# ardaduz/deep-video-mvs

Measured on NVIDIA H100. Metric: fusionnet depth frames/sec @256x256x64planes, higher is better.
Workload: dtype f16+f32acc

## Files before the change

### deep-video-mvs_b200/dvmvs/_blocks.py

```python
import torch

from . import _native as N
from . import _ops as ops
from ._base import NativeModule, auto_graph, pack_cbr, pack_head
from .config import Config
from .convlstm import MVSLayernormConvLSTMCell
from .layers import conv_layer, depth_layer_3x3

fpn_output_channels = 32
hyper_channels = 32

D, U = N.SRC_DIRECT, N.SRC_UPSAMPLE2X


class StandardLayer(NativeModule):
    def __init__(self, channels, kernel_size, apply_bn_relu):
        super().__init__()
        self.conv1 = conv_layer(channels, channels, kernel_size, 1, True)
        self.conv2 = conv_layer(channels, channels, kernel_size, 1, apply_bn_relu)

    def _pack(self):
        return ops.ConvLayer(pack_cbr(self.conv1)), ops.ConvLayer(pack_cbr(self.conv2))

    def run(self, x):
# ... 72 lines not shown
                depth = depth_producer()
                c1.prestage_upsampled(depth)
        x = self.up_convolution.run(x)
        if fork is not None:
            fork.join()
        srcs = [(x, D), (skip, D)] if depth is None else [(x, D), (skip, D), (depth, U)]
        h, w = x.f32.shape[1], x.f32.shape[2]
        blk_only = c1.path(h, w) == "halo" and c2.path(h, w) == "halo"
        y = c1.run(srcs, want_f32=not blk_only, want_planes=not blk_only)
        return c2.run([(y, D)], want_planes=False, want_blk=False)

    def forward(self, x, skip, depth):
        return ops.act_to_api(self.run(ops.to_act(x), ops.to_act(skip), None if depth is None else ops.to_act(depth)))


class _InvertedResidual(torch.nn.Module):

    def __init__(self, in_ch, out_ch, kernel_size, stride, expansion):
        super().__init__()
        mid = in_ch * expansion
        self.apply_residual = in_ch == out_ch and stride == 1
        self.stride = stride
        self.layers = torch.nn.Sequential(
            torch.nn.Conv2d(in_ch, mid, 1, bias=False), torch.nn.BatchNorm2d(mid), torch.nn.ReLU(inplace=True),
            torch.nn.Conv2d(mid, mid, kernel_size, padding=kernel_size // 2, stride=stride, groups=mid, bias=False),
            torch.nn.BatchNorm2d(mid), torch.nn.ReLU(inplace=True),
            torch.nn.Conv2d(mid, out_ch, 1, bias=False), torch.nn.BatchNorm2d(out_ch))


def _stack(in_ch, out_ch, kernel_size, stride, expansion, repeats):
    blocks = [_InvertedResidual(in_ch, out_ch, kernel_size, stride, expansion)]
    blocks += [_InvertedResidual(out_ch, out_ch, kernel_size, 1, expansion) for _ in range(repeats - 1)]
    return torch.nn.Sequential(*blocks)


class FeatureExtractor(NativeModule):

    def __init__(self):
        super().__init__()
        self.layer1 = torch.nn.Sequential(
            torch.nn.Conv2d(3, 32, 3, padding=1, stride=2, bias=False), torch.nn.BatchNorm2d(32), torch.nn.ReLU(inplace=True),
            torch.nn.Conv2d(32, 32, 3, padding=1, stride=1, groups=32, bias=False), torch.nn.BatchNorm2d(32), torch.nn.ReLU(inplace=True),
            torch.nn.Conv2d(32, 16, 1, padding=0, stride=1, bias=False), torch.nn.BatchNorm2d(16))
        self.layer2 = torch.nn.Sequential(_stack(16, 24, 3, 2, 3, 3))
        self.layer3 = torch.nn.Sequential(_stack(24, 40, 5, 2, 3, 3))
        self.layer4 = torch.nn.Sequential(_stack(40, 80, 5, 2, 6, 3), _stack(80, 96, 3, 1, 6, 2))
        self.layer5 = torch.nn.Sequential(_stack(96, 192, 5, 2, 6, 4), _stack(192, 320, 3, 1, 6, 1))

    def _pack(self):
        l1 = self.layer1
        stem = (ops.ConvLayer(ops.PackedConv(l1[0].weight, None, l1[1], stride=2, act=N.ACT_RELU)),
                ops.PackedDepthwise(l1[3].weight, l1[4], stride=1),
                ops.ConvLayer(ops.PackedConv(l1[6].weight, None, l1[7], stride=1, act=N.ACT_NONE)))
        levels = []
        for layer in (self.layer2, self.layer3, self.layer4, self.layer5):
            blocks = []
            for stack in layer:
                for blk in stack:
                    L = blk.layers
                    blocks.append((ops.ConvLayer(ops.PackedConv(L[0].weight, None, L[1], act=N.ACT_RELU)),
                                   ops.PackedDepthwise(L[3].weight, L[4], stride=blk.stride),
                                   ops.ConvLayer(ops.PackedConv(L[6].weight, None, L[7], act=N.ACT_NONE)), blk.apply_residual))
            levels.append(blocks)
        return stem, levels

    def run(self, x, image_nchw=None, part="all"):
        stem, levels = self.packed()
        def depthwise(t, dw, consumer):
            if consumer.uses_tc():
                return ops.Act(None, ops.dwconv2d(t.f32, dw, want_f32=False, want_planes=True)[1])
            return ops.Act(ops.dwconv2d(t.f32, dw))

        outs = []
        if part != "tail":
            if image_nchw is not None:
                x = ops.Act(ops.stem_conv(image_nchw, stem[0].pc))
            else:
                x = stem[0].run([(x, D)])
            x = depthwise(x, stem[1], stem[2])
            x = stem[2].run([(x, D)])
            outs = [x]
        for blocks in {"all": levels, "head": levels[:2], "tail": levels[2:]}[part]:
            for expand, dw, project, residual in blocks:
                y = depthwise(expand.run([(x, D)], want_planes=False), dw, project)
                x = project.run([(y, D)], residual=x if residual else None,
                                residual_mode=N.RES_SAME if residual else N.RES_NONE)
            outs.append(x)
        return outs

    @auto_graph
    @ops.family_terms("fe")
    def forward(self, image):
        B, C, H, W = image.shape
        if C != 3 or H % 32 != 0 or W % 32 != 0:
            raise RuntimeError("FeatureExtractor: expected (B,3,H,W) with H, W multiples of 32, got %s" % (tuple(image.shape),))
        ops.require_cuda_f32(image, "image")
        if image.is_contiguous():
            return tuple(ops.act_to_api(t) for t in self.run(None, image_nchw=image))
        return tuple(ops.act_to_api(t) for t in self.run(ops.to_act(image, "image")))

    @ops.family_terms("fe")
    def forward_head(self, image):
        ops.require_cuda_f32(image, "image")
        return tuple(ops.act_to_api(t) for t in self.run(None, image_nchw=image.contiguous(), part="head"))

    @ops.family_terms("fe")
    def forward_tail(self, head):
        l1, l2, l3 = head
        tail = self.run(ops.to_act(l3, "layer3"), part="tail")
        return (l1, l2, l3) + tuple(ops.act_to_api(t) for t in tail)


class _FPNHolder(torch.nn.Module):

    def __init__(self, in_channels_list, out_channels):
        super().__init__()
        self.inner_blocks = torch.nn.ModuleList([torch.nn.Conv2d(c, out_channels, 1) for c in in_channels_list])
        self.layer_blocks = torch.nn.ModuleList([torch.nn.Conv2d(out_channels, out_channels, 3, padding=1) for _ in in_channels_list])


class FeatureShrinker(NativeModule):

    def __init__(self):
        super().__init__()
        self.fpn = _FPNHolder([16, 24, 40, 96, 320], fpn_output_channels)

    def _pack(self):
        inner = [ops.ConvLayer(ops.PackedConv(m.weight, m.bias)) for m in self.fpn.inner_blocks]
        layer = [ops.ConvLayer(ops.PackedConv(m.weight, m.bias)) for m in self.fpn.layer_blocks]
        return inner, layer

    def run(self, feats):
        inner, layer = self.packed()
        last = inner[4].run([(feats[4], D)])
        outs = [None] * 4
        keep, forks = [last], []
        for i in (3, 2, 1, 0):
            last = inner[i].run([(feats[i], D)], residual=last, residual_mode=N.RES_NEAREST_UP)
            keep.append(last)
            if i > 0:
                f = ops.Fork()
                with f:
                    outs[i] = layer[i].run([(last, D)])
                forks.append(f)
            else:
                outs[i] = layer[i].run([(last, D)])
        for f in forks:
            f.join()
        del keep
        return outs

    @auto_graph
    @ops.family_terms("fpn")
    def forward(self, layer1, layer2, layer3, layer4, layer5):
        feats = [ops.to_act(t, "layer%d" % (i + 1)) for i, t in enumerate((layer1, layer2, layer3, layer4, layer5))]
        return tuple(ops.act_to_api(t) for t in self.run(feats))


class CostVolumeEncoder(NativeModule):
    def __init__(self):
        super().__init__()
        h = hyper_channels
        self.aggregator0 = conv_layer(Config.train_n_depth_levels + fpn_output_channels, h, 5, 1, True)
        self.encoder_block0 = EncoderBlock(h, h * 2, 5)
        self.aggregator1 = conv_layer(h * 2 + fpn_output_channels, h * 2, 3, 1, True)
        self.encoder_block1 = EncoderBlock(h * 2, h * 4, 3)
        self.aggregator2 = conv_layer(h * 4 + fpn_output_channels, h * 4, 3, 1, True)
# ... 113 lines not shown
```

### deep-video-mvs_b200/dvmvs/_native.py

```python
import ctypes
import os

_HERE = os.path.dirname(os.path.abspath(__file__))
LIB_PATH = os.path.join(os.path.dirname(_HERE), "lib", "libdvmvs_sm90.so")

c_float_p = ctypes.c_void_p
ABI_VERSION = 6
_lib = None

ACT_NONE, ACT_RELU, ACT_SIGMOID = 0, 1, 2
SRC_DIRECT, SRC_UPSAMPLE2X = 0, 1
SPLIT_UPSAMPLE2X, SPLIT_HI_ONLY = 1, 2
RES_NONE, RES_SAME, RES_NEAREST_UP = 0, 1, 2
SWEEP_DOT, SWEEP_SAD = 0, 1
LOSS_L1, LOSS_L1_INV, LOSS_L1_REL, LOSS_HUBER = 0, 1, 2, 3

EXPORTED_SYMBOLS = [
    "dvmvs_abi_version", "dvmvs_set_programmatic_launch", "dvmvs_last_error_string", "dvmvs_kernel_launch_count", "dvmvs_plane_sweep_fused",
    "dvmvs_hidden_warp", "dvmvs_depth_reproject", "dvmvs_conv2d", "dvmvs_conv2d_tc", "dvmvs_conv2d_halo", "dvmvs_split_blocked", "dvmvs_split_planes", "dvmvs_stem_conv", "dvmvs_dwconv2d", "dvmvs_lstm_gates",
    "dvmvs_upsample2x", "dvmvs_nchw_to_nhwc", "dvmvs_nhwc_to_nchw", "dvmvs_preprocess_rgb", "dvmvs_tsdf_integrate",
    "dvmvs_plane_sweep_backward", "dvmvs_hidden_warp_backward", "dvmvs_lstm_gates_backward", "dvmvs_depth_loss_forward",
    "dvmvs_depth_loss_backward", "dvmvs_plane_sweep_fused_h16", "dvmvs_plane_sweep_tc", "dvmvs_lstm_gates_parts", "dvmvs_conv2d_tc_ksplit", "dvmvs_plane_sweep_tc_set_timeline",
    "dvmvs_mesh_scratch_bytes", "dvmvs_mesh_count", "dvmvs_mesh_extract",
]


class ConvDesc(ctypes.Structure):
    _fields_ = [
        ("src", ctypes.c_void_p * 3), ("src_channels", ctypes.c_int * 3), ("src_mode", ctypes.c_int * 3),
        ("n_src", ctypes.c_int),
        ("weight", ctypes.c_void_p), ("bias", ctypes.c_void_p), ("residual", ctypes.c_void_p),
        ("residual_mode", ctypes.c_int), ("Hr", ctypes.c_int), ("Wr", ctypes.c_int),
        ("out", ctypes.c_void_p), ("aux_out", ctypes.c_void_p),
        ("aux_mult", ctypes.c_float), ("aux_base", ctypes.c_float),
        ("B", ctypes.c_int), ("Hin", ctypes.c_int), ("Win", ctypes.c_int), ("Cout", ctypes.c_int),
        ("ksize", ctypes.c_int), ("stride", ctypes.c_int), ("act", ctypes.c_int),
        ("workspace", ctypes.c_void_p), ("workspace_bytes", ctypes.c_longlong),
    ]


class ConvTcDesc(ctypes.Structure):
    _fields_ = [
        ("src_planes", ctypes.c_void_p * 3), ("src_channels", ctypes.c_int * 3), ("n_src", ctypes.c_int),
        ("w_hi", ctypes.c_void_p), ("w_lo", ctypes.c_void_p),
        ("w_rows", ctypes.c_int), ("ktot", ctypes.c_int), ("block_n", ctypes.c_int), ("terms", ctypes.c_int),
        ("allow_split", ctypes.c_int),
        ("bias", ctypes.c_void_p), ("residual", ctypes.c_void_p),
        ("residual_mode", ctypes.c_int), ("Hr", ctypes.c_int), ("Wr", ctypes.c_int),
        ("out_f32", ctypes.c_void_p), ("out_planes", ctypes.c_void_p), ("aux_out", ctypes.c_void_p),
        ("aux_mult", ctypes.c_float), ("aux_base", ctypes.c_float),
        ("B", ctypes.c_int), ("Hin", ctypes.c_int), ("Win", ctypes.c_int), ("Cout", ctypes.c_int),
        ("ksize", ctypes.c_int), ("stride", ctypes.c_int), ("act", ctypes.c_int),
        ("workspace", ctypes.c_void_p), ("workspace_bytes", ctypes.c_longlong),
        ("out_blk", ctypes.c_void_p),
        ("out_hi_only", ctypes.c_int), ("defer_finish", ctypes.c_int),
    ]


DRYRUN = os.environ.get("DVMVS_DRYRUN") == "1"


class _DryRunLib:

    def __getattr__(self, name):
        if name == "dvmvs_last_error_string":
            return lambda: b"dry run"
        if name == "dvmvs_kernel_launch_count":
            return lambda: 0
        return lambda *a, **k: 0


class ConvHaloDesc(ctypes.Structure):
    _fields_ = [
        ("src_blk", ctypes.c_void_p * 3), ("src_c8", ctypes.c_int * 3), ("n_src", ctypes.c_int),
        ("w_hi", ctypes.c_void_p), ("w_lo", ctypes.c_void_p),
        ("n_groups", ctypes.c_int), ("kc", ctypes.c_int), ("block_n", ctypes.c_int), ("terms", ctypes.c_int),
        ("bias", ctypes.c_void_p), ("residual", ctypes.c_void_p),
        ("out_f32", ctypes.c_void_p), ("out_blk", ctypes.c_void_p), ("out_nhwc", ctypes.c_void_p),
        ("B", ctypes.c_int), ("H", ctypes.c_int), ("W", ctypes.c_int), ("Cout", ctypes.c_int),
        ("ksize", ctypes.c_int), ("act", ctypes.c_int),
        ("w_cat", ctypes.c_void_p),
        ("out_hi_only", ctypes.c_int),
    ]


def lib():
    global _lib
    if _lib is None and DRYRUN:
        _lib = _DryRunLib()
    if _lib is None:
        if not os.path.isfile(LIB_PATH):
            raise RuntimeError("dvmvs: %s not found -- build it with `python deep-video-mvs_b200/build_native.py` "
                               "(there is no CPU / eager fallback)" % LIB_PATH)
        L = ctypes.CDLL(LIB_PATH)
        if L.dvmvs_abi_version() != ABI_VERSION:
            raise RuntimeError("dvmvs: %s has ABI version %d, this binding was written for %d -- rebuild it with "
                               "`python deep-video-mvs_b200/build_native.py --force`" % (LIB_PATH, L.dvmvs_abi_version(), ABI_VERSION))
        i, f, p = ctypes.c_int, ctypes.c_float, ctypes.c_void_p
        L.dvmvs_last_error_string.restype = ctypes.c_char_p
        L.dvmvs_set_programmatic_launch.argtypes = [i]
        L.dvmvs_plane_sweep_fused.argtypes = [p, p, p, p, p, p, i, i, i, i, i, i, f, f, i, p]
        L.dvmvs_plane_sweep_generic.argtypes = [p, p, p, p, p, p, i, i, i, i, i, i, f, f, i, p]
        L.dvmvs_plane_sweep_fused_h16.argtypes = [p, p, p, p, p, p, i, i, i, i, i, i, f, f, p]
        L.dvmvs_plane_sweep_tc.argtypes = [p, p, p, p, p, p, p, p, i, i, i, i, i, f, f, i, p]
        L.dvmvs_plane_sweep_tc_set_timeline.argtypes = [p]
        L.dvmvs_hidden_warp.argtypes = [p, p, p, p, p, p, i, i, i, i, f, p]
        L.dvmvs_depth_reproject.argtypes = [p, p, p, p, p, p, i, i, i, p]
        L.dvmvs_conv2d.argtypes = [ctypes.POINTER(ConvDesc), p]
        L.dvmvs_conv2d_tc.argtypes = [ctypes.POINTER(ConvTcDesc), p]
        L.dvmvs_conv2d_halo.argtypes = [ctypes.POINTER(ConvHaloDesc), p]
        L.dvmvs_split_blocked.argtypes = [p, p, i, i, i, i, i, i, i, i, p]
        L.dvmvs_split_planes.argtypes = [p, p, i, i, i, i, i, i, i, i, p]
        L.dvmvs_stem_conv.argtypes = [p, p, p, p, i, i, i, p]
        L.dvmvs_dwconv2d.argtypes = [p, p, p, p, p, i, i, i, i, i, i, i, p]
        L.dvmvs_lstm_gates.argtypes = [p, p, p, p, i, i, i, i, p]
        L.dvmvs_lstm_gates_parts.argtypes = [p, i, ctypes.c_longlong, p, p, p, p, i, i, i, i, p]
        L.dvmvs_conv2d_tc_ksplit.argtypes = [ctypes.POINTER(ConvTcDesc)]
        L.dvmvs_upsample2x.argtypes = [p, p, i, i, i, i, p]
        L.dvmvs_preprocess_rgb.argtypes = [p, i, i, i, i, i, i, p, i, i, i, f, ctypes.POINTER(ctypes.c_float), ctypes.POINTER(ctypes.c_float), p]
        L.dvmvs_nchw_to_nhwc.argtypes = [p, p, i, i, i, i, p]
        L.dvmvs_nhwc_to_nchw.argtypes = [p, p, i, i, i, i, p]
        d = ctypes.c_double
        L.dvmvs_tsdf_integrate.argtypes = [p, p, p, i, i, i, ctypes.POINTER(ctypes.c_float), d, d, p, i, p, i, i, i,
                                           ctypes.POINTER(ctypes.c_float), ctypes.POINTER(ctypes.c_double), d, p, p]
        ll = ctypes.c_longlong
        L.dvmvs_mesh_scratch_bytes.argtypes = [i, i, i, ctypes.POINTER(ll)]
        L.dvmvs_mesh_count.argtypes = [p, i, i, i, p, ll, p]
        L.dvmvs_mesh_extract.argtypes = [p, p, i, i, i, ctypes.POINTER(ctypes.c_float), f, p, ll, i, i, p, p, p, p, p, p]
        L.dvmvs_plane_sweep_backward.argtypes = [p, p, p, p, p, p, p, p, i, i, i, i, i, i, f, f, i, p]
        L.dvmvs_hidden_warp_backward.argtypes = [p, p, p, p, p, p, i, i, i, i, f, p]
        L.dvmvs_lstm_gates_backward.argtypes = [p, p, p, p, p, p, i, i, i, i, p]
        ip, fp = ctypes.POINTER(ctypes.c_int), ctypes.POINTER(ctypes.c_float)
        L.dvmvs_depth_loss_forward.argtypes = [p, ip, ip, i, p, p, i, i, i, p]
        L.dvmvs_depth_loss_backward.argtypes = [p, p, ip, ip, fp, i, p, p, p, i, i, i, i, p]
        _lib = L
    return _lib


def check(rc, what):
    if rc != 0:
        raise RuntimeError("dvmvs native call %s failed (%d): %s" % (what, rc, lib().dvmvs_last_error_string().decode()))


def launch_count():
    return lib().dvmvs_kernel_launch_count()
```

### deep-video-mvs_b200/dvmvs/_ops.py

```python
import ctypes
import os as _os_mod


def _os_environ_get(k, d):
    return _os_mod.environ.get(k, d)


import torch

from . import _native as N


def _stream():
    if N.DRYRUN:
        return None
    return ctypes.c_void_p(torch.cuda.current_stream().cuda_stream)


def _first_tensor(args):
    for a in args:
        if isinstance(a, torch.Tensor):
            return a
        if isinstance(a, (list, tuple)):
            t = _first_tensor(a)
# ... 389 lines not shown
        w2d = torch.zeros(rows, self.ktot, dtype=torch.float32)
        w2d[:cout] = wk.reshape(self.ktot, cout).t()
        hi = w2d.to(torch.float16)
        lo = (w2d - hi.to(torch.float32)).to(torch.float16)
        self.w_hi = hi.contiguous().to(device)
        self.w_lo = lo.contiguous().to(device)
        self.rows = rows
        self.ksize, self.cin, self.cout, self.stride, self.act = k, cin, cout, pc.stride, pc.act
        self.bias = pc.bias.to(device) if pc.bias is not None else None
        self.src_channels = list(src_channels)


@on_tensor_device
def conv2d_tc(sources, ptc, residual=None, residual_mode=N.RES_NONE, aux=None, want_f32=True, want_planes=True, terms=3,
              block_n=None, allow_split=True, blk_out=None, defer_finish=False):
    d = N.ConvTcDesc()
    first = sources[0]
    B, Hin, Win = first.shape[1], first.shape[2], first.shape[3]
    if len(sources) != len(ptc.src_stored):
        raise ValueError("conv2d_tc: %d sources given, weights packed for %d" % (len(sources), len(ptc.src_stored)))
    for i, t in enumerate(sources):
        if t.dtype != torch.float16 or tuple(t.shape[:4]) != (2, B, Hin, Win) or t.shape[4] != ptc.src_stored[i]:
            raise ValueError("conv2d_tc: source %d has shape %s / %s, expected (2,%d,%d,%d,%d) fp16"
                             % (i, tuple(t.shape), t.dtype, B, Hin, Win, ptc.src_stored[i]))
        d.src_planes[i] = t.data_ptr()
        d.src_channels[i] = t.shape[4]
    d.n_src = len(sources)
    pad = (ptc.ksize - 1) // 2
    Hout = (Hin + 2 * pad - ptc.ksize) // ptc.stride + 1
    Wout = (Win + 2 * pad - ptc.ksize) // ptc.stride + 1
    if block_n is None:
        tiles = B * ((Hout + 7) // 8) * ((Wout + 15) // 16)
        if ptc.cout >= 1024 and tiles < 16:
            block_n = 128
        elif ptc.cout <= 32 or tiles < 16:
            block_n = 32
        elif ptc.cout <= 64 or tiles < 64:
            block_n = 64
        else:
            block_n = 128
    if want_planes and ptc.cout % 8 != 0:
        raise ValueError("conv2d_tc: fp16-pair output needs Cout % 8 == 0")
    dev = first.device
    out_f32 = torch.empty((B, Hout, Wout, ptc.cout), dtype=torch.float32, device=dev) if want_f32 else None
    out_planes = torch.empty((2, B, Hout, Wout, ptc.cout), dtype=torch.float16, device=dev) if want_planes else None
    d.w_hi, d.w_lo = ptc.w_hi.data_ptr(), ptc.w_lo.data_ptr()
    d.w_rows, d.ktot, d.block_n, d.terms, d.allow_split = ptc.rows, ptc.ktot, block_n, terms, 1 if allow_split else 0
    d.bias = ptc.bias.data_ptr() if ptc.bias is not None else None
    d.residual_mode = residual_mode
    if residual is not None:
        d.residual = residual.data_ptr()
        d.Hr, d.Wr = residual.shape[1], residual.shape[2]
    d.out_f32 = out_f32.data_ptr() if out_f32 is not None else None
    d.out_planes = out_planes.data_ptr() if out_planes is not None else None
    if blk_out is not None:
        d.out_blk = blk_out.data_ptr()
    aux_out = None
    if aux is not None:
        aux_out = torch.empty((B, Hout, Wout, ptc.cout), dtype=torch.float32, device=dev)
        d.aux_out = aux_out.data_ptr()
        d.aux_mult, d.aux_base = aux
    d.B, d.Hin, d.Win, d.Cout = B, Hin, Win, ptc.cout
    d.ksize, d.stride, d.act = ptc.ksize, ptc.stride, ptc.act
    ws = None
    if allow_split:
        ws = workspace(dev)
        d.workspace, d.workspace_bytes = ws.data_ptr(), WORKSPACE_BYTES
    d.out_hi_only = 0 if lo_planes_needed() else 1
    if defer_finish:
        k = N.lib().dvmvs_conv2d_tc_ksplit(ctypes.byref(d)) if (ws is not None and not N.DRYRUN) else 1
        if k > 1 and residual is None and aux is None:
            d.defer_finish = 1
            d.out_f32 = d.out_planes = d.out_blk = None
            N.check(N.lib().dvmvs_conv2d_tc(ctypes.byref(d), _stream()), "conv2d_tc(deferred finish)")
            return ("parts", (ws, 16384, k, B * Hout * Wout * ptc.cout))
        return None
    N.check(N.lib().dvmvs_conv2d_tc(ctypes.byref(d), _stream()), "conv2d_tc")
    if aux is not None:
        return out_f32, out_planes, aux_out
    return out_f32, out_planes


@on_tensor_device
def split_blocked(sources, only=None, into=None):
    shp = lambda t: tuple(t) if isinstance(t, (tuple, list)) else tuple(t.shape)
    shapes = [(shp(t)[1] * (2 if up else 1), shp(t)[2] * (2 if up else 1)) for t, up in sources]
    B, (Ho, Wo) = shp(sources[0][0])[0], shapes[0]
    if any(sh != (Ho, Wo) for sh in shapes):
        raise ValueError("split_blocked: spatial sizes differ: %s" % (shapes,))
    C8 = sum((shp(t)[3] + 7) // 8 for t, _ in sources)
    if into is None:
        dev = next(t.device for t, _ in sources if isinstance(t, torch.Tensor))
        into = torch.empty((2, B, C8, Ho, Wo, 8), dtype=torch.float16, device=dev)
    planes = into
    hi_only = 0 if lo_planes_needed() else N.SPLIT_HI_ONLY
    off = 0
    for i, (t, up) in enumerate(sources):
        C = shp(t)[3]
        cover = (C + 7) // 8 * 8
        if only is None or i in only:
            flags = (N.SPLIT_UPSAMPLE2X if up else 0) | hi_only
            N.check(N.lib().dvmvs_split_blocked(t.data_ptr(), planes.data_ptr(), B, t.shape[1], t.shape[2], C, C8, flags, off, cover,
                                                _stream()), "split_blocked")
        off += cover
    return planes


class PackedConvHalo:

    def __init__(self, pc, src_channels, device, kc=None, block_n=None, concat_padded=False):
        k, cin, cout = pc.ksize, pc.cin, pc.cout
        assert sum(src_channels) == cin and pc.stride == 1
        self.kc = kc or (16 if k == 5 else 32)
        self.block_n = block_n or (32 if cout <= 32 else 64)
        kc, bn = self.kc, self.block_n
        w = pc.weight.detach().to("cpu", torch.float32)
        n_tiles = (cout + bn - 1) // bn
        if concat_padded:
            padded = torch.zeros(k, k, sum((c + 7) // 8 * 8 for c in src_channels), cout, dtype=torch.float32)
            src_off, dst_off = 0, 0
            for cr in src_channels:
                padded[:, :, dst_off:dst_off + cr, :] = w[:, :, src_off:src_off + cr, :]
                src_off, dst_off = src_off + cr, dst_off + (cr + 7) // 8 * 8
            w, src_channels = padded, [padded.shape[2]]
        groups = []
        self.src_c8 = []
        off = 0
        for cr in src_channels:
            c8 = (cr + 7) // 8
            self.src_c8.append(c8)
            for cg in range((c8 * 8 + kc - 1) // kc):
                lo_c = cg * kc
                groups.append((off + lo_c, max(0, min(kc, cr - lo_c))))
            off += cr
        self.n_groups = len(groups)
        packed = torch.zeros(n_tiles, self.n_groups, k, k, kc // 8, bn, 8, dtype=torch.float32)
        for gi, (c0, nvalid) in enumerate(groups):
            if nvalid == 0:
                continue
            blk = torch.zeros(k, k, kc, n_tiles * bn, dtype=torch.float32)
            blk[:, :, :nvalid, :cout] = w[:, :, c0:c0 + nvalid, :]
            blk = blk.reshape(k, k, kc // 8, 8, n_tiles, bn).permute(4, 0, 1, 2, 5, 3)
            packed[:, gi] = blk
        hi = packed.to(torch.float16)
        lo = (packed - hi.to(torch.float32)).to(torch.float16)
        self.w_hi, self.w_lo = hi.contiguous().to(device), lo.contiguous().to(device)
        self.ksize, self.cin, self.cout, self.act = k, cin, cout, pc.act
        self.bias = pc.bias.to(device) if pc.bias is not None else None
        self.src_channels = list(src_channels)


@on_tensor_device
def conv2d_halo(sources_blk, ph, residual=None, terms=3, want_f32=True, want_blk=False, want_nhwc=True):
    d = N.ConvHaloDesc()
    first = sources_blk[0]
    B, H, W = first.shape[1], first.shape[3], first.shape[4]
    if len(sources_blk) != len(ph.src_c8):
        raise ValueError("conv2d_halo: %d sources given, weights packed for %d" % (len(sources_blk), len(ph.src_c8)))
    for i, t in enumerate(sources_blk):
        if t.dtype != torch.float16 or tuple(t.shape) != (2, B, ph.src_c8[i], H, W, 8):
            raise ValueError("conv2d_halo: source %d has shape %s, expected %s" % (i, tuple(t.shape), (2, B, ph.src_c8[i], H, W, 8)))
        d.src_blk[i] = t.data_ptr()
        d.src_c8[i] = ph.src_c8[i]
    d.n_src = len(sources_blk)
    dev = first.device
    out_f32 = torch.empty((B, H, W, ph.cout), dtype=torch.float32, device=dev) if want_f32 else None
# ... 315 lines not shown
```

### include/dvmvs_b200.h

```cpp
#ifndef DVMVS_B200_H
#define DVMVS_B200_H

#include <stdint.h>

#ifdef __cplusplus
extern "C" {
#endif

typedef void* dvmvs_stream_t;

enum {
  DVMVS_OK = 0,
  DVMVS_EINVAL = -1,
  DVMVS_ELAUNCH = -2,
  DVMVS_EUNSUPPORTED = -3
};

enum { DVMVS_ACT_NONE = 0, DVMVS_ACT_RELU = 1, DVMVS_ACT_SIGMOID = 2 };
enum { DVMVS_SRC_DIRECT = 0, DVMVS_SRC_UPSAMPLE2X = 1 };
enum { DVMVS_SPLIT_UPSAMPLE2X = 1, DVMVS_SPLIT_HI_ONLY = 2 };
enum { DVMVS_RES_NONE = 0, DVMVS_RES_SAME = 1, DVMVS_RES_NEAREST_UP = 2 };
enum { DVMVS_SWEEP_DOT = 0, DVMVS_SWEEP_SAD = 1 };
enum { DVMVS_LOSS_L1 = 0, DVMVS_LOSS_L1_INV = 1, DVMVS_LOSS_L1_REL = 2, DVMVS_LOSS_HUBER = 3 };

// ... 20 lines not shown
int dvmvs_hidden_warp(const float* h_in, const float* depth, const float* prev_pose, const float* cur_pose,
                      const float* K, float* h_out, int B, int C, int h, int w, float invalid_thresh,
                      dvmvs_stream_t stream);

int dvmvs_depth_reproject(const float* cur_pose, const float* prev_pose, const float* prev_depth,
                          const float* full_K, const float* half_K, float* out, int B, int H, int W,
                          dvmvs_stream_t stream);

typedef struct {
  const float* src[3];
  int src_channels[3];
  int src_mode[3];
  int n_src;
  const float* weight;
  const float* bias;
  const float* residual;
  int residual_mode, Hr, Wr;
  float* out;
  float* aux_out;
  float aux_mult, aux_base;
  int B, Hin, Win, Cout, ksize, stride, act;
  float* workspace;
  long long workspace_bytes;
} dvmvs_conv_desc;

int dvmvs_conv2d(const dvmvs_conv_desc* desc_host, dvmvs_stream_t stream);

typedef struct {
  const void* src_planes[3];
  int src_channels[3];
  int n_src;
  const void* w_hi;
  const void* w_lo;
  int w_rows, ktot, block_n, terms, allow_split;
  const float* bias;
  const float* residual;
  int residual_mode, Hr, Wr;
  float* out_f32;
  void* out_planes;
  float* aux_out;
  float aux_mult, aux_base;
  int B, Hin, Win, Cout, ksize, stride, act;
  float* workspace;
  long long workspace_bytes;
  void* out_blk;
  int out_hi_only;
  int defer_finish;
} dvmvs_conv_tc_desc;

int dvmvs_conv2d_tc(const dvmvs_conv_tc_desc* desc_host, dvmvs_stream_t stream);
int dvmvs_conv2d_tc_ksplit(const dvmvs_conv_tc_desc* desc_host);

typedef struct {
  const void* src_blk[3];
  int src_c8[3];
  int n_src;
  const void* w_hi;
  const void* w_lo;
  int n_groups, kc, block_n, terms;
  const float* bias;
  const float* residual;
  float* out_f32;
  void* out_blk;
  void* out_nhwc;
  int B, H, W, Cout, ksize, act;
  const void* w_cat;
  int out_hi_only;
} dvmvs_conv_halo_desc;

int dvmvs_conv2d_halo(const dvmvs_conv_halo_desc* desc_host, dvmvs_stream_t stream);

int dvmvs_split_blocked(const float* x, void* planes, int B, int H, int W, int C, int C8, int flags, int c_offset,
                        int c_cover, dvmvs_stream_t stream);

int dvmvs_split_planes(const float* x, void* planes, int B, int H, int W, int C, int Cs, int upsample2x, int c_offset,
                       int c_cover, dvmvs_stream_t stream);

int dvmvs_stem_conv(const float* image_nchw, const float* weight, const float* bias, float* y, int B, int H, int W,
                    dvmvs_stream_t stream);

int dvmvs_dwconv2d(const float* x, const float* weight, const float* bias, float* y, void* y_planes, int B, int H, int W,
                   int C, int ksize, int stride, int act, dvmvs_stream_t stream);

int dvmvs_lstm_gates(const float* gates, const float* c_in, float* h_out, float* c_out, int B, int h, int w, int C,
                     dvmvs_stream_t stream);

int dvmvs_lstm_gates_parts(const float* gate_parts, int n_parts, long long part_stride, const float* addend, const float* c_in,
                           float* h_out, float* c_out, int B, int h, int w, int C, dvmvs_stream_t stream);

int dvmvs_upsample2x(const float* x, float* y, int B, int H, int W, int C, dvmvs_stream_t stream);

int dvmvs_preprocess_rgb(const void* image, int is_u8, int swap_rb, int in_h, int in_w, int crop_x, int crop_y, float* out,
                         int out_h, int out_w, int normalize, float scale, const float* mean3, const float* std3,
                         dvmvs_stream_t stream);


int dvmvs_plane_sweep_backward(const float* ref, const float* const* meas_host, const float* pose1,
                               const float* const* pose2_host, const float* K, const float* grad_cost, float* grad_ref,
                               float* const* grad_meas_host, int B, int C, int h, int w, int D, int M, float min_depth,
                               float max_depth, int mode, dvmvs_stream_t stream);

int dvmvs_hidden_warp_backward(const float* grad_out, const float* depth, const float* prev_pose, const float* cur_pose,
                               const float* K, float* grad_h_in, int B, int C, int h, int w, float invalid_thresh,
                               dvmvs_stream_t stream);

int dvmvs_lstm_gates_backward(const float* gates, const float* c_in, const float* grad_h, const float* grad_c, float* grad_gates,
                              float* grad_c_in, int B, int h, int w, int C, dvmvs_stream_t stream);

int dvmvs_depth_loss_forward(const float* const* preds_host, const int* hs_host, const int* ws_host, int n_scales,
                             const float* groundtruth, float* sums, int B, int H, int W, dvmvs_stream_t stream);

int dvmvs_depth_loss_backward(const float* const* preds_host, float* const* grads_host, const int* hs_host, const int* ws_host,
                              const float* weights_host, int n_scales, const float* groundtruth, const float* sums,
                              const float* upstream, int loss_type, int B, int H, int W, dvmvs_stream_t stream);

int dvmvs_nchw_to_nhwc(const float* x, float* y, int B, int C, int H, int W, dvmvs_stream_t stream);
int dvmvs_nhwc_to_nchw(const float* x, float* y, int B, int C, int H, int W, dvmvs_stream_t stream);

int dvmvs_tsdf_integrate(float* tsdf_vol, float* weight_vol, float* color_vol, int dim_x, int dim_y, int dim_z,
                         const float* vol_origin3, double voxel_size, double trunc_margin, const void* color_im,
                         int color_is_u8, const void* depth_im, int depth_is_f64, int im_h, int im_w, const float* intr4,
                         const double* world_to_cam16, double obs_weight, unsigned long long* updated_count,
                         dvmvs_stream_t stream);

int dvmvs_mesh_scratch_bytes(int dim_x, int dim_y, int dim_z, long long* bytes_host);
int dvmvs_mesh_count(const float* tsdf_vol, int dim_x, int dim_y, int dim_z, void* scratch, long long scratch_bytes,
                     dvmvs_stream_t stream);
int dvmvs_mesh_extract(const float* tsdf_vol, const float* color_vol, int dim_x, int dim_y, int dim_z,
                       const float* vol_origin_host, float voxel_size, const void* scratch, long long scratch_bytes, int n_verts,
                       int n_faces, int* vertex_keys, float* verts, int* faces, float* norms, unsigned char* colors,
                       dvmvs_stream_t stream);

#ifdef __cplusplus
}
#endif
#endif
```

Before: 1738.

## Fuse 1x1 expansion GEMM with depthwise conv in feature-extractor blocks

```diff
diff --git a/deep-video-mvs_b200/csrc/expand_dw.cu b/deep-video-mvs_b200/csrc/expand_dw.cu
--- /dev/null
+++ b/deep-video-mvs_b200/csrc/expand_dw.cu
@@ -0,0 +1,254 @@
+#include <string.h>
+
+#include "tc_ptx.cuh"
+
+namespace dvmvs {
+
+constexpr int kEdThreads = 256;
+constexpr int kEdSmemBudget = 113 * 1024;
+
+struct ExpandDwParams {
+  CUtensorMap a_map[2];
+  CUtensorMap w_map[2];
+  int kc, n_chunks, terms, write_lo;
+  int B, H, W, mid, Ho, Wo, stride, pad;
+  int tile_h, tile_w, tiles_x, tiles_y, halo_h, halo_w, n_halo, m_blocks;
+  const float* e_bias;
+  int e_act;
+  const float* dw_w;
+  const float* dw_b;
+  int dw_act;
+  __half* out;
+  int a_chunk_bytes, w_chunk_bytes, a_bytes, w_bytes, tile_off;
+};
+
+template <int BLOCK_N, int KSTEPS>
+__device__ __forceinline__ void ed_mma_block(float (&acc)[BLOCK_N / 2], const ExpandDwParams& p, uint32_t a_base, uint32_t w_base, int mb) {
+  constexpr uint32_t layout = (KSTEPS == 4) ? kGmmaSw128 : kGmmaSw64;
+  constexpr uint32_t row_bytes = KSTEPS * 32u;
+  constexpr uint32_t sbo = 8u * row_bytes;
+  wgmma_fence_regs(acc);
+  wgmma_fence();
+  for (int ch = 0; ch < p.n_chunks; ++ch) {
+    for (int term = 0; term < p.terms; ++term) {
+      const uint32_t a_s = a_base + ((term == 1) ? p.a_bytes : 0u) + ch * p.a_chunk_bytes + mb * 64u * row_bytes;
+      const uint32_t w_s = w_base + ((term == 2) ? p.w_bytes : 0u) + ch * p.w_chunk_bytes;
+#pragma unroll
+      for (int k = 0; k < KSTEPS; ++k)
+        wgmma_f16<BLOCK_N>(acc, gmma_desc(a_s + 32u * k, 16u, sbo, layout), gmma_desc(w_s + 32u * k, 16u, sbo, layout));
+    }
+  }
+  wgmma_commit();
+  wgmma_wait<0>();
+  wgmma_fence_regs(acc);
+}
+
+template <int BLOCK_N, int KS>
+__global__ void __launch_bounds__(kEdThreads, 2) expand_dw_kernel(const __grid_constant__ ExpandDwParams p) {
+  pdl_launch_dependents();
+  extern __shared__ uint8_t smem_raw[];
+  const uint32_t raw_addr = smem_u32(smem_raw);
+  const uint32_t base = (raw_addr + 1023u) & ~1023u;
+  uint8_t* base_ptr = smem_raw + (base - raw_addr);
+  const uint32_t planes = p.terms > 1 ? 2u : 1u;
+  const uint32_t a_base = base, w_base = base + planes * p.a_bytes;
+  float* tile = reinterpret_cast<float*>(base_ptr + p.tile_off);
+  const uint32_t bar = base + p.tile_off + ((p.n_halo * (BLOCK_N + 4) * 4 + 7) & ~7);
+  constexpr int kPitch = BLOCK_N + 4;
+
+  const int tiles_per_img = p.tiles_x * p.tiles_y;
+  const int b = blockIdx.x / tiles_per_img;
+  const int t_in = blockIdx.x - b * tiles_per_img;
+  const int oy0 = (t_in / p.tiles_x) * p.tile_h, ox0 = (t_in % p.tiles_x) * p.tile_w;
+  const int c0 = blockIdx.y * BLOCK_N;
+
+  if (threadIdx.x == 0) {
+    asm volatile("prefetch.tensormap [%0];" ::"l"(&p.a_map[0]) : "memory");
+    if (p.terms > 1) asm volatile("prefetch.tensormap [%0];" ::"l"(&p.a_map[1]) : "memory");
+    mbar_init(bar, 1);
+    asm volatile("fence.mbarrier_init.release.cluster;" ::: "memory");
+  }
+  __syncthreads();
+  pdl_wait();
+
+  if (threadIdx.x == 0) {
+    mbar_expect_tx(bar, planes * p.n_chunks * (p.n_halo * p.kc * 2 + BLOCK_N * p.kc * 2));
+    const int iy = oy0 * p.stride - p.pad, ix = ox0 * p.stride - p.pad;
+    for (uint32_t pl = 0; pl < planes; ++pl)
+      for (int ch = 0; ch < p.n_chunks; ++ch) {
+        tma_load_4d(a_base + pl * p.a_bytes + ch * p.a_chunk_bytes, &p.a_map[pl], bar, ch * p.kc, ix, iy, b);
+        tma_load_2d(w_base + pl * p.w_bytes + ch * p.w_chunk_bytes, &p.w_map[pl], bar, ch * p.kc, c0);
+      }
+  }
+  mbar_wait(bar, 0);
+
+  const int wg = threadIdx.x >> 7, warp = (threadIdx.x >> 5) & 3, lane = threadIdx.x & 31;
+  for (int mb = wg; mb < p.m_blocks; mb += 2) {
+    float acc[BLOCK_N / 2];
+#pragma unroll
+    for (int i = 0; i < BLOCK_N / 2; ++i) acc[i] = 0.f;
+    if (p.kc == 64) ed_mma_block<BLOCK_N, 4>(acc, p, a_base, w_base, mb);
+    else ed_mma_block<BLOCK_N, 2>(acc, p, a_base, w_base, mb);
+    const int r0 = mb * 64 + warp * 16 + (lane >> 2);
+#pragma unroll
+    for (int j = 0; j < BLOCK_N / 8; ++j) {
+      const int c = 8 * j + 2 * (lane & 3);
+      const float b0 = (c0 + c < p.mid) ? __ldg(p.e_bias + c0 + c) : 0.f;
+      const float b1 = (c0 + c + 1 < p.mid) ? __ldg(p.e_bias + c0 + c + 1) : 0.f;
+#pragma unroll
+      for (int h = 0; h < 2; ++h) {
+        const int r = r0 + 8 * h;
+        if (r < p.n_halo)
+          *reinterpret_cast<float2*>(tile + r * kPitch + c) =
+              make_float2(tc_act(acc[4 * j + 2 * h] + b0, p.e_act), tc_act(acc[4 * j + 2 * h + 1] + b1, p.e_act));
+      }
+    }
+  }
+  __syncthreads();
+
+  const int groups = (min(BLOCK_N, p.mid - c0)) >> 3;
+  const size_t plane_stride = (size_t)p.B * p.Ho * p.Wo * p.mid;
+#pragma unroll 1
+  for (int item = threadIdx.x; item < p.tile_h * p.tile_w * groups; item += kEdThreads) {
+    const int pix = item / groups, g = item - pix * groups;
+    const int ty = pix / p.tile_w, tx = pix - ty * p.tile_w;
+    const int oy = oy0 + ty, ox = ox0 + tx;
+    if (oy >= p.Ho || ox >= p.Wo) continue;
+    const int c = c0 + 8 * g;
+    float acc[8];
+    *reinterpret_cast<float4*>(acc) = __ldg(reinterpret_cast<const float4*>(p.dw_b + c));
+    *reinterpret_cast<float4*>(acc + 4) = __ldg(reinterpret_cast<const float4*>(p.dw_b + c + 4));
+#pragma unroll
+    for (int ky = 0; ky < KS; ++ky) {
+      const int iy = oy * p.stride - p.pad + ky;
+      const bool yok = iy >= 0 && iy < p.H;
+#pragma unroll
+      for (int kx = 0; kx < KS; ++kx) {
+        const int ix = ox * p.stride - p.pad + kx;
+        if (!(yok && ix >= 0 && ix < p.W)) continue;
+        const float* xp = tile + ((ty * p.stride + ky) * p.halo_w + tx * p.stride + kx) * kPitch + 8 * g;
+        float xv[8], wv[8];
+        *reinterpret_cast<float4*>(xv) = *reinterpret_cast<const float4*>(xp);
+        *reinterpret_cast<float4*>(xv + 4) = *reinterpret_cast<const float4*>(xp + 4);
+        const float* wp = p.dw_w + (size_t)(ky * KS + kx) * p.mid + c;
+        *reinterpret_cast<float4*>(wv) = __ldg(reinterpret_cast<const float4*>(wp));
+        *reinterpret_cast<float4*>(wv + 4) = __ldg(reinterpret_cast<const float4*>(wp + 4));
+#pragma unroll
+        for (int e = 0; e < 8; ++e) acc[e] = fmaf(xv[e], wv[e], acc[e]);
+      }
+    }
+    __align__(16) __half hi[8];
+    __align__(16) __half lo[8];
+#pragma unroll
+    for (int e = 0; e < 8; ++e) {
+      const float v = (p.dw_act == DVMVS_ACT_RELU) ? fmaxf(acc[e], 0.f) : acc[e];
+      hi[e] = __float2half_rn(v);
+      lo[e] = __float2half_rn(v - __half2float(hi[e]));
+    }
+    __half* o = p.out + (((size_t)b * p.Ho + oy) * p.Wo + ox) * p.mid + c;
+    *reinterpret_cast<uint4*>(o) = *reinterpret_cast<const uint4*>(hi);
+    if (p.write_lo) *reinterpret_cast<uint4*>(o + plane_stride) = *reinterpret_cast<const uint4*>(lo);
+  }
+}
+
+static int ed_smem_bytes(int th, int tw, int k, int s, int kc, int n_chunks, int terms, int block_n, int* n_halo, int* m_blocks) {
+  const int hh = (th - 1) * s + k, hw = (tw - 1) * s + k;
+  *n_halo = hh * hw;
+  *m_blocks = (*n_halo + 63) / 64;
+  const int planes = terms > 1 ? 2 : 1;
+  const int a = planes * n_chunks * (*m_blocks * 64 * kc * 2), w = planes * n_chunks * block_n * kc * 2;
+  return 1024 + a + w + ((*n_halo * (block_n + 4) * 4 + 7) & ~7) + 8;
+}
+
+template <int BLOCK_N, int KS>
+static int launch_ed(const ExpandDwParams& p, dim3 grid, int smem, cudaStream_t s) {
+  static PerDeviceOnce attr_set;
+  if (attr_set.first()) {
+    cudaError_t e = cudaFuncSetAttribute(expand_dw_kernel<BLOCK_N, KS>, cudaFuncAttributeMaxDynamicSharedMemorySize, 227 * 1024);
+    if (e != cudaSuccess) { set_error("expand_dw smem attribute: %s", cudaGetErrorString(e)); return DVMVS_ELAUNCH; }
+  }
+  launch_k(expand_dw_kernel<BLOCK_N, KS>, grid, dim3(kEdThreads), (size_t)smem, s, p);
+  return check_launch("expand_dw_kernel");
+}
+
+}
+
+using namespace dvmvs;
+
+extern "C" int dvmvs_expand_dwconv(const void* x_planes, int B, int H, int W, int Cs, const void* w_hi, const void* w_lo, int w_rows, int ktot,
+                                   const float* expand_bias, int expand_act, const float* dw_weight, const float* dw_bias, int ksize,
+                                   int stride, int dw_act, int mid, int terms, int write_lo, void* y_planes, dvmvs_stream_t stream) {
+  DVMVS_REQUIRE(tensor_map_encoder() != nullptr, "expand_dwconv: cuTensorMapEncodeTiled entry point not available");
+  DVMVS_REQUIRE(x_planes && w_hi && (terms == 1 || w_lo) && expand_bias && dw_weight && dw_bias && y_planes, "expand_dwconv: null pointer");
+  DVMVS_REQUIRE(B > 0 && H > 0 && W > 0 && Cs > 0 && Cs % 8 == 0 && mid > 0 && mid % 8 == 0,
+                "expand_dwconv: bad shape (B=%d H=%d W=%d Cs=%d mid=%d; Cs and mid must be multiples of 8)", B, H, W, Cs, mid);
+  DVMVS_REQUIRE((ksize == 3 || ksize == 5) && (stride == 1 || stride == 2), "expand_dwconv: ksize=%d stride=%d", ksize, stride);
+  DVMVS_REQUIRE(terms == 1 || terms == 3, "expand_dwconv: terms=%d", terms);
+  DVMVS_REQUIRE(expand_act == DVMVS_ACT_NONE || expand_act == DVMVS_ACT_RELU, "expand_dwconv: expand act %d", expand_act);
+  DVMVS_REQUIRE(dw_act == DVMVS_ACT_NONE || dw_act == DVMVS_ACT_RELU, "expand_dwconv: depthwise act %d", dw_act);
+  DVMVS_REQUIRE((uintptr_t)x_planes % 16 == 0 && (uintptr_t)w_hi % 16 == 0 && (uintptr_t)w_lo % 16 == 0 && (uintptr_t)dw_weight % 16 == 0 &&
+                    (uintptr_t)dw_bias % 16 == 0 && (uintptr_t)y_planes % 16 == 0,
+                "expand_dwconv: pointers must be 16-byte aligned");
+  ExpandDwParams p;
+  memset(&p, 0, sizeof(p));
+  p.kc = (Cs % 64 == 0) ? 64 : 32;
+  p.n_chunks = (Cs + p.kc - 1) / p.kc;
+  DVMVS_REQUIRE(ktot == p.n_chunks * p.kc, "expand_dwconv: packed weight K=%d, expected %d", ktot, p.n_chunks * p.kc);
+  const int block_n = ((mid + 31) / 32 * 32 < (mid + 63) / 64 * 64) ? 32 : 64;
+  const int n_slices = (mid + block_n - 1) / block_n;
+  DVMVS_REQUIRE(w_rows % block_n == 0 && w_rows >= n_slices * block_n, "expand_dwconv: weight rows %d do not cover %d channels", w_rows, mid);
+  p.terms = terms; p.write_lo = write_lo ? 1 : 0;
+  p.B = B; p.H = H; p.W = W; p.mid = mid; p.stride = stride; p.pad = ksize / 2;
+  p.Ho = (H + 2 * p.pad - ksize) / stride + 1;
+  p.Wo = (W + 2 * p.pad - ksize) / stride + 1;
+  static const int cands[4][2] = {{8, 16}, {8, 8}, {4, 8}, {4, 4}};
+  const int n_sms = device_sm_count();
+  int smem = 0;
+  bool chosen = false;
+  for (int i = 0; i < 4; ++i) {
+    const int th = min(cands[i][0], p.Ho), tw = min(cands[i][1], p.Wo);
+    int n_halo, m_blocks;
+    const int bytes = ed_smem_bytes(th, tw, ksize, stride, p.kc, p.n_chunks, terms, block_n, &n_halo, &m_blocks);
+    if (bytes > kEdSmemBudget && i < 3) continue;
+    const int tiles = ((p.Ho + th - 1) / th) * ((p.Wo + tw - 1) / tw);
+    p.tile_h = th; p.tile_w = tw; p.tiles_y = (p.Ho + th - 1) / th; p.tiles_x = (p.Wo + tw - 1) / tw;
+    p.halo_h = (th - 1) * stride + ksize; p.halo_w = (tw - 1) * stride + ksize;
+    p.n_halo = n_halo; p.m_blocks = m_blocks;
+    smem = bytes;
+    chosen = true;
+    if ((long long)B * tiles * n_slices >= 2LL * n_sms) break;
+  }
+  DVMVS_REQUIRE(chosen && smem <= 227 * 1024, "expand_dwconv: no tile fits shared memory (Cs=%d mid=%d k=%d)", Cs, mid, ksize);
+  const int planes = terms > 1 ? 2 : 1;
+  p.a_chunk_bytes = p.m_blocks * 64 * p.kc * 2;
+  p.w_chunk_bytes = block_n * p.kc * 2;
+  p.a_bytes = p.n_chunks * p.a_chunk_bytes;
+  p.w_bytes = p.n_chunks * p.w_chunk_bytes;
+  p.tile_off = planes * (p.a_bytes + p.w_bytes);
+  p.e_bias = expand_bias; p.e_act = expand_act;
+  p.dw_w = dw_weight; p.dw_b = dw_bias; p.dw_act = dw_act;
+  p.out = (__half*)y_planes;
+  const size_t plane = (size_t)B * H * W * Cs;
+  for (int pl = 0; pl < planes; ++pl) {
+    const void* xp = (const __half*)x_planes + pl * plane;
+    cuuint64_t dims[4] = {(cuuint64_t)Cs, (cuuint64_t)W, (cuuint64_t)H, (cuuint64_t)B};
+    cuuint64_t strides[3] = {(cuuint64_t)Cs * 2, (cuuint64_t)W * Cs * 2, (cuuint64_t)H * W * Cs * 2};
+    cuuint32_t box[4] = {(cuuint32_t)p.kc, (cuuint32_t)p.halo_w, (cuuint32_t)p.halo_h, 1};
+    cuuint32_t estr[4] = {1, 1, 1, 1};
+    const CUtensorMapSwizzle sw = p.kc == 64 ? CU_TENSOR_MAP_SWIZZLE_128B : CU_TENSOR_MAP_SWIZZLE_64B;
+    CUresult r = cached_tensor_map(&p.a_map[pl], CU_TENSOR_MAP_DATA_TYPE_FLOAT16, 4, xp, dims, strides, box, estr, sw,
+                                   CU_TENSOR_MAP_L2_PROMOTION_L2_128B);
+    DVMVS_REQUIRE(r == CUDA_SUCCESS, "expand_dwconv: cuTensorMapEncodeTiled(activation) failed: %d", (int)r);
+    cuuint64_t wdims[2] = {(cuuint64_t)ktot, (cuuint64_t)w_rows};
+    cuuint64_t wstrides[1] = {(cuuint64_t)ktot * 2};
+    cuuint32_t wbox[2] = {(cuuint32_t)p.kc, (cuuint32_t)block_n};
+    cuuint32_t westr[2] = {1, 1};
+    r = cached_tensor_map(&p.w_map[pl], CU_TENSOR_MAP_DATA_TYPE_FLOAT16, 2, pl ? w_lo : w_hi, wdims, wstrides, wbox, westr, sw,
+                          CU_TENSOR_MAP_L2_PROMOTION_L2_256B);
+    DVMVS_REQUIRE(r == CUDA_SUCCESS, "expand_dwconv: cuTensorMapEncodeTiled(weights) failed: %d", (int)r);
+  }
+  const dim3 grid(p.tiles_x * p.tiles_y * B, n_slices);
+  cudaStream_t s = (cudaStream_t)stream;
+  if (block_n == 32) return ksize == 3 ? launch_ed<32, 3>(p, grid, smem, s) : launch_ed<32, 5>(p, grid, smem, s);
+  return ksize == 3 ? launch_ed<64, 3>(p, grid, smem, s) : launch_ed<64, 5>(p, grid, smem, s);
+}
diff --git a/deep-video-mvs_b200/dvmvs/_blocks.py b/deep-video-mvs_b200/dvmvs/_blocks.py
--- a/deep-video-mvs_b200/dvmvs/_blocks.py
+++ b/deep-video-mvs_b200/dvmvs/_blocks.py
@@ -178,7 +178,10 @@
             outs = [x]
         for blocks in {"all": levels, "head": levels[:2], "tail": levels[2:]}[part]:
             for expand, dw, project, residual in blocks:
-                y = depthwise(expand.run([(x, D)], want_planes=False), dw, project)
+                if expand.uses_tc():
+                    y = ops.Act(None, ops.expand_dwconv(x, expand, dw))
+                else:
+                    y = depthwise(expand.run([(x, D)], want_planes=False), dw, project)
                 x = project.run([(y, D)], residual=x if residual else None,
                                 residual_mode=N.RES_SAME if residual else N.RES_NONE)
             outs.append(x)
diff --git a/deep-video-mvs_b200/dvmvs/_native.py b/deep-video-mvs_b200/dvmvs/_native.py
--- a/deep-video-mvs_b200/dvmvs/_native.py
+++ b/deep-video-mvs_b200/dvmvs/_native.py
@@ -17,7 +17,7 @@
 
 EXPORTED_SYMBOLS = [
     "dvmvs_abi_version", "dvmvs_set_programmatic_launch", "dvmvs_last_error_string", "dvmvs_kernel_launch_count", "dvmvs_plane_sweep_fused",
-    "dvmvs_hidden_warp", "dvmvs_depth_reproject", "dvmvs_conv2d", "dvmvs_conv2d_tc", "dvmvs_conv2d_halo", "dvmvs_split_blocked", "dvmvs_split_planes", "dvmvs_stem_conv", "dvmvs_dwconv2d", "dvmvs_lstm_gates",
+    "dvmvs_hidden_warp", "dvmvs_depth_reproject", "dvmvs_conv2d", "dvmvs_conv2d_tc", "dvmvs_conv2d_halo", "dvmvs_split_blocked", "dvmvs_split_planes", "dvmvs_stem_conv", "dvmvs_dwconv2d", "dvmvs_expand_dwconv", "dvmvs_lstm_gates",
     "dvmvs_upsample2x", "dvmvs_nchw_to_nhwc", "dvmvs_nhwc_to_nchw", "dvmvs_preprocess_rgb", "dvmvs_tsdf_integrate",
     "dvmvs_plane_sweep_backward", "dvmvs_hidden_warp_backward", "dvmvs_lstm_gates_backward", "dvmvs_depth_loss_forward",
     "dvmvs_depth_loss_backward", "dvmvs_plane_sweep_fused_h16", "dvmvs_plane_sweep_tc", "dvmvs_lstm_gates_parts", "dvmvs_conv2d_tc_ksplit", "dvmvs_plane_sweep_tc_set_timeline",
@@ -113,6 +113,7 @@
         L.dvmvs_split_planes.argtypes = [p, p, i, i, i, i, i, i, i, i, p]
         L.dvmvs_stem_conv.argtypes = [p, p, p, p, i, i, i, p]
         L.dvmvs_dwconv2d.argtypes = [p, p, p, p, p, i, i, i, i, i, i, i, p]
+        L.dvmvs_expand_dwconv.argtypes = [p, i, i, i, i, p, p, i, i, p, i, p, p, i, i, i, i, i, i, p, p]
         L.dvmvs_lstm_gates.argtypes = [p, p, p, p, i, i, i, i, p]
         L.dvmvs_lstm_gates_parts.argtypes = [p, i, ctypes.c_longlong, p, p, p, p, i, i, i, i, p]
         L.dvmvs_conv2d_tc_ksplit.argtypes = [ctypes.POINTER(ConvTcDesc)]
diff --git a/deep-video-mvs_b200/dvmvs/_ops.py b/deep-video-mvs_b200/dvmvs/_ops.py
--- a/deep-video-mvs_b200/dvmvs/_ops.py
+++ b/deep-video-mvs_b200/dvmvs/_ops.py
@@ -495,6 +495,31 @@
 
 
 @on_tensor_device
+def expand_dwconv(act, expand_layer, dw, terms=None):
+    terms = _TC_TERMS if terms is None else int(terms)
+    pc = expand_layer.pc
+    if pc.ksize != 1 or pc.stride != 1 or not expand_layer.tc_eligible() or dw.channels != pc.cout:
+        raise ValueError("expand_dwconv: needs a tensor-core 1x1 expansion to %d channels, got k=%d stride=%d cout=%d"
+                         % (dw.channels, pc.ksize, pc.stride, pc.cout))
+    if expand_layer._ptc is None:
+        expand_layer._ptc = PackedConvTC(pc, expand_layer.src_channels, pc.weight.device)
+    ptc = expand_layer._ptc
+    x = act.get_planes()
+    _, B, H, W, Cs = x.shape
+    if Cs != ptc.src_stored[0]:
+        raise ValueError("expand_dwconv: input has %d channels, weights packed for %d" % (Cs, ptc.src_stored[0]))
+    pad = dw.ksize // 2
+    Hout = (H + 2 * pad - dw.ksize) // dw.stride + 1
+    Wout = (W + 2 * pad - dw.ksize) // dw.stride + 1
+    planes = torch.empty((2, B, Hout, Wout, dw.channels), dtype=torch.float16, device=x.device)
+    N.check(N.lib().dvmvs_expand_dwconv(x.data_ptr(), B, H, W, Cs, ptc.w_hi.data_ptr(), ptc.w_lo.data_ptr(), ptc.rows, ptc.ktot,
+                                        ptc.bias.data_ptr(), ptc.act, dw.weight.data_ptr(), dw.bias.data_ptr(), dw.ksize, dw.stride,
+                                        dw.act, dw.channels, terms, 1 if terms == 3 else 0, planes.data_ptr(), _stream()),
+            "expand_dwconv")
+    return planes
+
+
+@on_tensor_device
 def split_blocked(sources, only=None, into=None):
     shp = lambda t: tuple(t) if isinstance(t, (tuple, list)) else tuple(t.shape)
     shapes = [(shp(t)[1] * (2 if up else 1), shp(t)[2] * (2 if up else 1)) for t, up in sources]
diff --git a/include/dvmvs_b200.h b/include/dvmvs_b200.h
--- a/include/dvmvs_b200.h
+++ b/include/dvmvs_b200.h
@@ -126,6 +126,10 @@
 int dvmvs_dwconv2d(const float* x, const float* weight, const float* bias, float* y, void* y_planes, int B, int H, int W,
                    int C, int ksize, int stride, int act, dvmvs_stream_t stream);
 
+int dvmvs_expand_dwconv(const void* x_planes, int B, int H, int W, int Cs, const void* w_hi, const void* w_lo, int w_rows, int ktot,
+                        const float* expand_bias, int expand_act, const float* dw_weight, const float* dw_bias, int ksize, int stride,
+                        int dw_act, int mid, int terms, int write_lo, void* y_planes, dvmvs_stream_t stream);
+
 int dvmvs_lstm_gates(const float* gates, const float* c_in, float* h_out, float* c_out, int B, int h, int w, int C,
                      dvmvs_stream_t stream);
 
```

Measured after the change: 1835, median of 6. +5.5%, better.
